# michelerenzullo/Blur_algorithms

Hardware: AMD Instinct MI355X
Metric: megapixels/sec Gaussian blur (σ=20, 4K RGB) at 1/2/4/8 GPUs; % HBM roofline (higher is better)
Workload: dtype f16 hi+lo operands (u8 pixels exact, taps and intermediate split in two binary16 halves), f32 accumulate

## Files before the change

blur_algorithms_amd/csrc/engine.hip:

```cpp
#include <hip/hip_runtime.h>

#include <array>
#include <cmath>
#include <cstdio>
#include <cstdlib>
#include <cstring>
#include <functional>
#include <list>
#include <map>
#include <memory>
#include <string>
#include <tuple>
#include <type_traits>
#include <vector>

#include "../../include/blur_amd.h"
#include "fast_registry.hpp"
#include "fft_engine.hpp"
#include "host_math.hpp"
#define BLUR_MX_QUIRK_KERNELS
#include "mx_registry.hpp"
#define BLUR_FX_QUIRK_KERNELS
#include "fx_registry.hpp"
#include "bx_box.hpp"
// ... 2608 lines not shown
        g.nframes = nf;
        g.aligned = ((cols & 3) == 0 && (reinterpret_cast<uintptr_t>(s) & 3) == 0) ? 1 : 0;
        int* spart = nullptr;
        float *vpart = nullptr, *qrow = nullptr, *qcol = nullptr;
        double* zpart = nullptr;
        if (p.mx_quirk) {
            spart = ctx->mx_sums;
            zpart = reinterpret_cast<double*>(ctx->mx_terms);
            vpart = reinterpret_cast<float*>(zpart + n_zpart * nf);
            qrow = vpart + n_vpart * nf;
            qcol = qrow + n_qrow * nf;
        }
        { TimedLaunch t(ctx, 0, nf);
          HIP_TRY(ctx, p.mx->row_u8(ctx->stream, s, ctx->work, p.mxt->frags_row, g, ctx->num_cus, spart, vpart)); }
        if (p.mx_quirk) {
            hipLaunchKernelGGL(mx_quirk_rows, dim3(zblocks, nf), dim3(256), 0, ctx->stream, spart, qrow, zpart, g, chunks, 8 * (p.mx->nkb - 2), p.mxt->dr);
            HIP_TRY(ctx, hipGetLastError());
            hipLaunchKernelGGL(mx_quirk_cols, dim3((g.vpitch + 255) / 256, nf), dim3(256), 0, ctx->stream, vpart, zpart, qcol, g, rblocks, zblocks, p.mxt->dr, p.mxt->dc);
            HIP_TRY(ctx, hipGetLastError());
        }
        { TimedLaunch t(ctx, 1, nf);
          HIP_TRY(ctx, p.mx->col_u8(ctx->stream, ctx->work, d, p.mxt->frags_col, g, qcol, ctx->num_cus, qrow)); }
    }
    return BLUR_OK;
}

static int run_fx_u8c3(blur_ctx* ctx, const uint8_t* d_src, uint8_t* d_dst, int nframes, int rows, int cols, const Prepared& p, float* vdump = nullptr, FwChSel chsel = 0,
                       const ChLayout* lay = nullptr, const FwFrame* ft)
{
    const size_t px = static_cast<size_t>(rows) * cols;
    if (lay && !chsel) return fail(ctx, BLUR_ERR_INVALID, "run_fx_u8c3: a layout goes with a channel selection");
    if (ft && !lay) return fail(ctx, BLUR_ERR_INVALID, "run_fx_u8c3: a frame list goes with a layout");
    const FwPitch pt = lay ? fw_pitch_of(*lay) : fw_pitch_packed(rows, cols, 3, 1);
    const uint8_t* lo = d_src < d_dst ? d_src : d_dst;
    const uint8_t* hi = d_src < d_dst ? d_dst : d_src;
    if (!lay && static_cast<size_t>(hi - lo) < px * 3 * nframes) {
        const size_t cap = std::max<size_t>(1, (static_cast<size_t>(1) << 30) / (px * 3));
        if (d_src == d_dst && static_cast<size_t>(nframes) > cap) {
            for (int f0 = 0; f0 < nframes; f0 += static_cast<int>(cap)) {
                const int nf = std::min<int>(static_cast<int>(cap), nframes - f0);
                if (int rc = run_fx_u8c3(ctx, d_src + static_cast<size_t>(f0) * px * 3, d_dst + static_cast<size_t>(f0) * px * 3, nf, rows, cols, p, vdump, chsel)) return rc;
            }
            return BLUR_OK;
        }
        if (int rc = ensure_work(ctx, px * 3 * nframes)) return rc;
        HIP_TRY(ctx, hipMemcpyAsync(ctx->work, d_src, px * 3 * nframes, hipMemcpyDeviceToDevice, ctx->stream));
        d_src = reinterpret_cast<const uint8_t*>(ctx->work);
    }
    const int nkb = p.fx->nkb, pada = 8 * (nkb - 2);
    FxGeom g{ rows, cols, p.sz.pad, nframes, 0, (rows + 31) / 32, fx_right_strips(cols, pada), ctx->num_xcds };
    g.aligned = ((cols & 3) == 0 && (reinterpret_cast<uintptr_t>(d_src) & 3) == 0 && (reinterpret_cast<uintptr_t>(d_dst) & 3) == 0) ? 1 : 0;
    {
        const int win = kFxChunk + 2 * pada, nstrips = fx_left_strips(pada) + g.nright;
        const size_t bytes = static_cast<size_t>(nframes) * nstrips * rows * win * 3 + 64;
        if (ctx->fx_strips_bytes < bytes) {
            if (ctx->fx_strips) { HIP_TRY(ctx, hipStreamSynchronize(ctx->stream)); HIP_TRY(ctx, hipFree(ctx->fx_strips)); ctx->fx_strips = nullptr; ctx->fx_strips_bytes = 0; }
            HIP_TRY(ctx, hipMalloc(reinterpret_cast<void**>(&ctx->fx_strips), bytes));
            ctx->fx_strips_bytes = bytes;
        }
    }
    const int chunks_x = (cols + kFxChunk - 1) / kFxChunk, narrow =
#ifdef FX_FULL_STRIPS
        0;
#else
        p.fx->nkb <= 11 && !chsel ? 1 : 0;
#endif
    int strip_groups = (kFxChunk + 2 * pada) / 4;
    if (narrow) {
        const int gpr = strip_groups, per = (gpr + 7) / 8, nleft = fx_left_strips(pada);
        strip_groups = 0;
        for (int si = 0; si < nleft + g.nright; ++si) {
            int lo, hi;
            fx_strip_range(si < nleft ? si : chunks_x - g.nright + si - nleft, cols, pada, per, &lo, &hi);
            strip_groups = std::max(strip_groups, std::min(8 * hi, gpr) - 8 * lo);
        }
        if (strip_groups < 1) strip_groups = 1;
    }
    const int strip_blocks = (((rows + 3) / 4) * strip_groups + 255) / 256;
    const int n_strip = strip_blocks * (fx_left_strips(pada) + g.nright) * nframes;
    FxQuirk qk{};
    if (!p.mx_quirk) {
        TimedLaunch t(ctx, 1, nframes);
        if (ft)
            hipLaunchKernelGGL(fx_prepass_frames<1>, dim3(n_strip), dim3(256), 0, ctx->stream, d_src, nullptr, nullptr, nullptr, ctx->fx_strips, rows, cols, pada, 1, 1, 0,
                               chunks_x, g.nright, strip_blocks, kFxSumRows, narrow, pt.src_pitch, pt.src_frame, ft);
        else
            hipLaunchKernelGGL(fx_prepass<1>, dim3(n_strip), dim3(256), 0, ctx->stream, d_src, nullptr, nullptr, nullptr, ctx->fx_strips, rows, cols, p.sz.pad, pada, 1, 1, 0,
                               chunks_x, g.nright, strip_blocks, kFxSumRows, narrow, pt.src_pitch, pt.src_frame);
        HIP_TRY(ctx, hipGetLastError());
    }
    if (p.mx_quirk) {
        const int gpt = fx_groups_per_thread(cols);
        const int groups = (cols + 3) / 4;
        const int band_rows = fx_band_rows(rows, cols, nframes, ctx->num_cus), nbands = (rows + band_rows - 1) / band_rows, nbatches = (groups + 256 * gpt - 1) / (256 * gpt);
        auto up4 = [](size_t v) { return (v + 3) & ~static_cast<size_t>(3); };
        const size_t n_srow = up4(static_cast<size_t>(nframes) * nbatches * rows * 3), n_cpart = up4(static_cast<size_t>(nframes) * nbands * 12 * groups);
        const size_t n_z = static_cast<size_t>(nframes) * nbands * nbatches * 3;
        const size_t bytes = (n_srow + n_cpart) * sizeof(int) + n_z * sizeof(long long) + 64;
        if (ctx->fx_sums_bytes < bytes) {
            if (ctx->fx_sums) { HIP_TRY(ctx, hipStreamSynchronize(ctx->stream)); HIP_TRY(ctx, hipFree(ctx->fx_sums)); ctx->fx_sums = nullptr; ctx->fx_sums_bytes = 0; }
            HIP_TRY(ctx, hipMalloc(reinterpret_cast<void**>(&ctx->fx_sums), bytes + bytes / 8));
            ctx->fx_sums_bytes = bytes + bytes / 8;
        }
        int* srow = ctx->fx_sums;
        int* cpart = srow + n_srow;
        long long* zpart = reinterpret_cast<long long*>(cpart + n_cpart);
        { TimedLaunch t(ctx, 1, nframes);
          const int n_alt = nbands * nbatches * nframes;
          auto kern = gpt == 1 ? fx_prepass<1> : (gpt == 2 ? fx_prepass<2> : fx_prepass<4>);
          auto kern_frames = gpt == 1 ? fx_prepass_frames<1> : (gpt == 2 ? fx_prepass_frames<2> : fx_prepass_frames<4>);
          if (ft)
              hipLaunchKernelGGL(kern_frames, dim3(n_alt + n_strip), dim3(256), 0, ctx->stream, d_src, srow, cpart, zpart, ctx->fx_strips, rows, cols, pada, nbands, nbatches,
                                 n_alt, chunks_x, g.nright, strip_blocks, band_rows, narrow, pt.src_pitch, pt.src_frame, ft);
          else
              hipLaunchKernelGGL(kern, dim3(n_alt + n_strip), dim3(256), 0, ctx->stream, d_src, srow, cpart, zpart, ctx->fx_strips, rows, cols, p.sz.pad, pada, nbands,
                                 nbatches, n_alt, chunks_x, g.nright, strip_blocks, band_rows, narrow, pt.src_pitch, pt.src_frame);
          HIP_TRY(ctx, hipGetLastError()); }
        qk.srow_part = srow;
        qk.cpart = cpart;
        qk.zpart = zpart;
        qk.taps = p.mxt->taps_row;
        qk.nbatches = nbatches;
        qk.nbands = nbands;
        qk.cpitch = 12 * groups;
        qk.dr = p.mxt->dr;
        qk.dc = p.mxt->dc;
    }
    unsigned long long* stamps = nullptr;
    if (!p.mx_quirk && !vdump && std::getenv("BLUR_FX_STAMPS")) {
        HIP_TRY(ctx, hipMalloc(reinterpret_cast<void**>(&stamps), 64));
        HIP_TRY(ctx, hipMemset(stamps, 0, 64));
    }
    if (chsel) {
        const Fw3Entry* fe3 = find_fw3_entry(nkb);
        if (!fe3 || vdump || stamps) return fail(ctx, BLUR_ERR_UNSUPPORTED, "fused kernel for a subset of three channels: no kernel instantiated for this pad");
        TimedLaunch t(ctx, 0, nframes);
        HIP_TRY(ctx, fe3->blur_u8(ctx->stream, d_src, d_dst, p.mxt->frags_row, g, ctx->num_cus, p.mx_quirk ? &qk : nullptr, ctx->fx_strips, chsel, pt, ft));
        return BLUR_OK;
    }
    { TimedLaunch t(ctx, 0, nframes);
      HIP_TRY(ctx, p.fx->blur_u8(ctx->stream, d_src, d_dst, p.mxt->frags_row, g, ctx->num_cus, p.mx_quirk ? &qk : nullptr, ctx->fx_strips, vdump, stamps)); }
    if (stamps) {
        unsigned long long h[8];
        HIP_TRY(ctx, hipStreamSynchronize(ctx->stream));
        HIP_TRY(ctx, hipMemcpy(h, stamps, 64, hipMemcpyDeviceToHost));
        HIP_TRY(ctx, hipFree(stamps));
        if (h[7]) {
            std::fprintf(stderr, "fx stamps: steps %llu, cycles per step: A0 %.0f B0 %.0f A1 %.0f B1 %.0f A2 %.0f B2 %.0f, whole task %.0f per step\n", h[7], h[0] / double(h[7]),
                         h[1] / double(h[7]), h[2] / double(h[7]), h[3] / double(h[7]), h[4] / double(h[7]), h[5] / double(h[7]), h[6] / double(h[7]));
        }
    }
    return BLUR_OK;
}

static bool bands_overlap(const uint8_t* lo, const uint8_t* hi, size_t bytes) { return static_cast<size_t>(hi - lo) < bytes; }

static int run_wr_tiled(blur_ctx* ctx, const uint8_t* d_src, uint8_t* d_dst, int nframes, int rows, int cols, const Prepared& p)
{
    const size_t px = static_cast<size_t>(rows) * cols, fb = px * 3;
    const int pad = p.sz.pad;
    const int groups = (cols + 3) / 4, gpt = 1;
    if (p.tl_quirk && cols < 4) return fail(ctx, BLUR_ERR_UNSUPPORTED, "tiled wave-resident path: image narrower than 4 pixels (the quirk's pre-pass)");
    const int pitch = (cols + 7) & ~7;
    int *srow = nullptr, *cpart = nullptr;
    long long* zpart = nullptr;
    float *e = nullptr, *h = nullptr;
    int band_rows = 0, nbands = 0, nbatches = 0;
    if (p.tl_quirk) {
        band_rows = static_cast<long long>(rows) * cols < 4000000ll ? 16 : kFxSumRows;
        while (band_rows < 256 && static_cast<long long>((groups + 255) / 256) * ((rows + 2 * band_rows - 1) / (2 * band_rows)) >= 4ll * ctx->num_cus) band_rows *= 2;
        nbands = (rows + band_rows - 1) / band_rows;
        nbatches = (groups + 256 * gpt - 1) / (256 * gpt);
        auto up4 = [](size_t v) { return (v + 3) & ~static_cast<size_t>(3); };
        const size_t n_srow = up4(static_cast<size_t>(nbatches) * rows * 3), n_cpart = up4(static_cast<size_t>(nbands) * 12 * groups);
        const size_t n_z = static_cast<size_t>(nbands) * nbatches * 3;
        const size_t bytes = (n_srow + n_cpart) * sizeof(int) + n_z * sizeof(long long) + 64;
        if (ctx->tl_sums_bytes < bytes) {
            if (ctx->tl_sums) { HIP_TRY(ctx, hipStreamSynchronize(ctx->stream)); HIP_TRY(ctx, hipFree(ctx->tl_sums)); ctx->tl_sums = nullptr; ctx->tl_sums_bytes = 0; }
            HIP_TRY(ctx, hipMalloc(reinterpret_cast<void**>(&ctx->tl_sums), bytes));
            ctx->tl_sums_bytes = bytes;
        }
        srow = ctx->tl_sums;
        cpart = srow + n_srow;
        zpart = reinterpret_cast<long long*>(cpart + n_cpart);
        const size_t tbytes = (static_cast<size_t>(3) * pitch + static_cast<size_t>(3) * rows) * sizeof(float) + 64;
        if (ctx->tl_terms_bytes < tbytes) {
            if (ctx->tl_terms) { HIP_TRY(ctx, hipStreamSynchronize(ctx->stream)); HIP_TRY(ctx, hipFree(ctx->tl_terms)); ctx->tl_terms = nullptr; ctx->tl_terms_bytes = 0; }
            HIP_TRY(ctx, hipMalloc(reinterpret_cast<void**>(&ctx->tl_terms), tbytes));
            ctx->tl_terms_bytes = tbytes;
        }
        e = ctx->tl_terms;
        h = e + static_cast<size_t>(3) * pitch;
    }
    for (int f = 0; f < nframes; ++f) {
        const uint8_t* src = d_src + static_cast<size_t>(f) * fb;
        uint8_t* dst = d_dst + static_cast<size_t>(f) * fb;
        const uint8_t* lo = src < dst ? src : dst;
        const uint8_t* hi = src < dst ? dst : src;
        if (bands_overlap(lo, hi, fb) && (p.bands.size() > 1 || p.tiles.size() > 1 || src == dst)) {
            if (ctx->tl_copy_bytes < fb) {
                if (ctx->tl_copy) { HIP_TRY(ctx, hipStreamSynchronize(ctx->stream)); HIP_TRY(ctx, hipFree(ctx->tl_copy)); ctx->tl_copy = nullptr; ctx->tl_copy_bytes = 0; }
                HIP_TRY(ctx, hipMalloc(reinterpret_cast<void**>(&ctx->tl_copy), fb));
                ctx->tl_copy_bytes = fb;
            }
            HIP_TRY(ctx, hipMemcpyAsync(ctx->tl_copy, src, fb, hipMemcpyDeviceToDevice, ctx->stream));
            src = ctx->tl_copy;
        }
        if (p.tl_quirk) {
            TimedLaunch t(ctx, 1, 1);
            const int n_alt = nbands * nbatches;
            hipLaunchKernelGGL(fx_prepass<1>, dim3(n_alt), dim3(256), 0, ctx->stream, src, srow, cpart, zpart, nullptr, rows, cols, pad, 0, nbands, nbatches, n_alt, 1, 0, 1, band_rows, 0,
                               static_cast<uint32_t>(cols) * 3u, static_cast<size_t>(rows) * cols * 3);
            HIP_TRY(ctx, hipGetLastError());
            const int ne = (pitch + 255) / 256, nh = (rows + 255) / 256;
            const size_t lds = (static_cast<size_t>(3) * (256 + 2 * pad) + (2 * pad + 1) + 3 + 3 * 256) * sizeof(double);
            if (lds > 64 * 1024) HIP_TRY(ctx, hipFuncSetAttribute(reinterpret_cast<const void*>(tl_terms_kernel), hipFuncAttributeMaxDynamicSharedMemorySize, static_cast<int>(lds)));
            hipLaunchKernelGGL(tl_terms_kernel, dim3(ne + nh, 1), dim3(256), lds, ctx->stream, srow, cpart, zpart, p.tl_taps, e, h, rows, cols, pad, pitch, nbatches, nbands,
                               12 * groups, p.tl_dr, p.tl_dc, ne);
            HIP_TRY(ctx, hipGetLastError());
        }
        auto group_of = [&](size_t bi, int& step) -> int {
            const Prepared::Span& b = p.bands[bi];
            const int brows = b.in1 - b.in0;
            int nb = 1;
            step = 0;
            if (b.padmode == 0) {
                while (bi + nb < p.bands.size()) {
                    const Prepared::Span& c = p.bands[bi + nb];
                    const int st = c.in0 - p.bands[bi + nb - 1].in0;
                    if (c.padmode != 0 || c.in1 - c.in0 != brows || c.v0 - c.in0 != b.v0 - b.in0 || c.v1 - c.v0 != b.v1 - b.v0 || (st & 1) || (nb > 1 && st != step)) break;
                    step = st;
                    ++nb;
                }
            }
            if (nb > 1 && wr_frame_floats(brows, cols, b.padmode, p.tl_col->g) * nb * sizeof(float) > (static_cast<size_t>(3) << 30)) { nb = 1; step = 0; }
            return nb;
        };
        {
            size_t need = 0;
            for (size_t bi = 0; bi < p.bands.size();) {
                int step;
                const int nb = group_of(bi, step);
                need = std::max(need, wr_frame_floats(p.bands[bi].in1 - p.bands[bi].in0, cols, p.bands[bi].padmode, p.tl_col->g) * nb * sizeof(float));
                bi += nb;
            }
            if (int rc = ensure_work(ctx, need)) return rc;
        }
        float* const inter = reinterpret_cast<float*>(ctx->work);
        for (size_t bi = 0; bi < p.bands.size();) {
            const Prepared::Span& b = p.bands[bi];
            const int brows = b.in1 - b.in0;
            int step = 0;
            const int nb = group_of(bi, step);
            const int vr_max = bi + nb < p.bands.size() ? p.bands[bi + nb].v0 : rows;
            WrColTerm term;
            if (p.tl_quirk) {
                term.e = e;
                term.pitch = pitch;
                term.sign = ((b.in0 + pad - b.padmode) & 1) ? -1.f : 1.f;
            }
            term.band_step = nb > 1 ? step : 0;
            { TimedLaunch t(ctx, 1, 1);
              HIP_TRY(ctx, p.tl_col->col_u8(ctx->stream, src + static_cast<size_t>(b.in0) * cols * 3, inter, brows, cols, b.padmode, nb, ctx->num_cus, ctx->d_w256, p.tl_tw0_col,
                                            p.tl_m_col, term)); }
            const int g = p.tl_col->g, npairs = wr_npairs(brows, b.padmode), strips_full = (cols + g - 1) / g;
            for (size_t ti = 0; ti < p.tiles.size(); ++ti) {
                const Prepared::Span& t = p.tiles[ti];
                WrRowTile tile;
                tile.h = p.tl_quirk ? h : nullptr;
                tile.rows_full = rows;
                tile.row_base = b.in0;
                tile.vr0 = b.v0;
                tile.vr1 = b.v1;
                tile.ypar = b.padmode & 1;
                tile.dst_pitch = cols * 3;
                tile.dst_x0 = t.in0;
                tile.vc0 = t.v0 - t.in0;
                tile.vc1 = t.v1 - t.in0;
                tile.xpar = (t.in0 + pad) & 1;
                tile.plane_strips = strips_full;
                tile.g = g;
                tile.t0 = (b.v0 - b.in0 + tile.ypar) >> 1;
                tile.tn = ((b.v1 - 1 - b.in0 + tile.ypar) >> 1) - tile.t0 + 1;
                tile.band_step = nb > 1 ? step : 0;
                tile.vr_max = vr_max;
                if (nb == 1 && tile.vr1 > vr_max) tile.vr1 = vr_max;
                TimedLaunch tl(ctx, 0, 1);
                HIP_TRY(ctx, p.tl_row[ti]->row_u8(ctx->stream, inter + static_cast<size_t>(t.in0 / g) * npairs * (2 * g), dst, brows, t.in1 - t.in0, t.padmode, nb, ctx->num_cus,
                                                  ctx->d_w256, p.tl_tw0_row[ti], p.tl_m_row[ti], tile));
            }
            bi += nb;
        }
    }
    return BLUR_OK;
// ... 1353 lines not shown
```

blur_algorithms_amd/csrc/fw_kernels.hpp:

```cpp
#pragma once
#include "fx_kernels.hpp"
#include <cstddef>
#include <type_traits>

#ifndef FW_TL_REGS
#define FW_TL_REGS 12
#endif

namespace blur_amd {

typedef uint32_t FwChSel;
constexpr FwChSel fw_chsel_all(int ch) { return static_cast<FwChSel>(ch) | (ch > 1 ? 0xe40u : 0u); }
inline FwChSel fw_chsel_mask(unsigned mask, int ch)
{
    FwChSel s = 0;
    int n = 0;
    for (int c = 0; c < ch; ++c)
        if (mask >> c & 1u) s |= static_cast<FwChSel>(c) << (4 + 2 * n++);
    return s | static_cast<FwChSel>(n);
}
__host__ __device__ constexpr int fw_chsel_count(FwChSel s) { return static_cast<int>(s & 7u); }
inline unsigned fw_chsel_bits(FwChSel s)
{
    unsigned m = 0;
// ... 567 lines not shown
                for (int j = 0; j < G; ++j)
                    d[i][j] = __builtin_amdgcn_raw_buffer_load_b32(rimg, dj[j] < ndw ? roff + 4u * dj[j] - back[j] : 0xfffffff0u, 0, 0) >> (8 * back[j]);
            }
#pragma unroll
            for (int i = 0; i < RB; ++i) {
                const int r = rb + i;
                if (r >= re) break;
                const int wy = mx_alt_weight(r, rows, pad);
                int s[CH];
#pragma unroll
                for (int ch = 0; ch < CH; ++ch) s[ch] = 0;
#pragma unroll
                for (int j = 0; j < G; ++j)
#pragma unroll
                    for (int k = 0; k < 4; ++k) {
                        const int v = wx[j][k] != 0 ? static_cast<int>((d[i][j] >> (8 * k)) & 0xffu) : 0;
                        s[CH == 1 ? 0 : k % CH] += wx[j][k] * v;
                        col[j][k] += wy * v;
                    }
#pragma unroll
                for (int ch = 0; ch < CH; ++ch)
                    if (chmask >> ch & 1u) atomicAdd(&sred[r - rs][ch][tid & 63], s[ch]);
            }
        }
        __syncthreads();
        if (tid < (re - rs) * CH && (chmask >> (tid % CH) & 1u)) {
            const int rr = tid / CH, ch = tid - rr * CH;
            const int* p64 = &sred[rr][ch][0];
            int v = 0;
#pragma unroll 8
            for (int k = 0; k < 64; ++k) v += p64[(k + tid) & 63];
            atomicAdd(&srow[(static_cast<size_t>(f) * rows + rs + rr) * CH + ch], v);
            atomicAdd(reinterpret_cast<unsigned long long*>(&zsum[static_cast<size_t>(f) * CH + ch]),
                      static_cast<unsigned long long>(static_cast<long long>(mx_alt_weight(rs + rr, rows, pad)) * v));
        }
        __syncthreads();
    }
#pragma unroll
    for (int j = 0; j < G; ++j)
        if (4 * dj[j] < cpitch)
            *reinterpret_cast<int4*>(cpart + (static_cast<size_t>(f) * nbands + band) * cpitch + 4 * dj[j]) = make_int4(col[j][0], col[j][1], col[j][2], col[j][3]);
}

template <int CH, int G>
__global__ __launch_bounds__(256) void fc_prepass(const uint8_t* __restrict__ src, int* __restrict__ srow, int* __restrict__ cpart, long long* __restrict__ zsum,
                                                  uint8_t* __restrict__ strips, int rows, int cols, int pad, int pada, int nbands, int nbatches, int cpitch, int n_alt,
                                                  int chunks, int nright, int strip_blocks, int band_rows, unsigned chmask, uint32_t spitch, size_t sframe)
{
    __shared__ int sred[kFcSumRows][CH][64];
    int b = blockIdx.x;
    if (b < n_alt) {
        const int band = b % nbands, batch = (b / nbands) % nbatches, f = b / (nbands * nbatches);
        fc_altsums_body<CH, G>(src, srow, cpart, zsum, rows, cols, pad, nbands, cpitch, band, batch, f, sred, band_rows, chmask, spitch, sframe);
    } else {
        b -= n_alt;
        const int nstrips = fx_left_strips(pada) + nright, bx = b % strip_blocks, sidx = (b / strip_blocks) % nstrips, f = b / (strip_blocks * nstrips);
        fc_edge_strips_body<CH>(src, strips, rows, cols, pada, chunks, nright, bx, sidx, f, spitch, sframe);
    }
}

template <int CH, int G>
__global__ __launch_bounds__(256) void fc_prepass_frames(const uint8_t* __restrict__ src, int* __restrict__ srow, int* __restrict__ cpart, long long* __restrict__ zsum,
                                                         uint8_t* __restrict__ strips, int rows, int cols, int pada, int nbands, int nbatches, int cpitch, int n_alt,
                                                         int chunks, int nright, int strip_blocks, int band_rows, unsigned chmask, uint32_t spitch, size_t sframe,
                                                         const FwFrame* __restrict__ ft)
{
    __shared__ int sred[kFcSumRows][CH][64];
    int b = blockIdx.x;
    if (b < n_alt) {
        const int band = b % nbands, batch = (b / nbands) % nbatches, f = b / (nbands * nbatches);
        const uint8_t* s = src + (static_cast<ptrdiff_t>(ft[f].frame) - f) * static_cast<ptrdiff_t>(sframe);
        fc_altsums_body<CH, G>(s, srow, cpart, zsum, rows, cols, ft[f].pad, nbands, cpitch, band, batch, f, sred, band_rows, chmask, spitch, sframe);
    } else {
        b -= n_alt;
        const int nstrips = fx_left_strips(pada) + nright, bx = b % strip_blocks, sidx = (b / strip_blocks) % nstrips, f = b / (strip_blocks * nstrips);
        const uint8_t* s = src + (static_cast<ptrdiff_t>(ft[f].frame) - f) * static_cast<ptrdiff_t>(sframe);
        fc_edge_strips_body<CH>(s, strips, rows, cols, pada, chunks, nright, bx, sidx, f, spitch, sframe);
    }
}

#ifdef BLUR_FX_QUIRK_KERNELS
template <int G>
__global__ __launch_bounds__(256) void fx_prepass_frames(const uint8_t* __restrict__ src, int* __restrict__ srow_part, int* __restrict__ cpart, long long* __restrict__ zpart,
                                                         uint8_t* __restrict__ strips, int rows, int cols, int pada, int nbands, int nbatches, int n_alt, int chunks,
                                                         int nright, int strip_blocks, int band_rows, int narrow, uint32_t spitch, size_t sframe,
                                                         const FwFrame* __restrict__ ft)
{
    __shared__ int sred[kFxSumRows][3][64];
    int b = blockIdx.x;
    if (b < n_alt) {
        const int band = b % nbands, batch = (b / nbands) % nbatches, f = b / (nbands * nbatches);
        const uint8_t* s = src + (static_cast<ptrdiff_t>(ft[f].frame) - f) * static_cast<ptrdiff_t>(sframe);
        fx_altsums_body<G>(s, srow_part, cpart, zpart, rows, cols, ft[f].pad, nbands, nbatches, band, batch, f, sred, band_rows, spitch, sframe);
    } else {
        b -= n_alt;
        const int nstrips = fx_left_strips(pada) + nright, bx = b % strip_blocks, sidx = (b / strip_blocks) % nstrips, f = b / (strip_blocks * nstrips);
        const uint8_t* s = src + (static_cast<ptrdiff_t>(ft[f].frame) - f) * static_cast<ptrdiff_t>(sframe);
        fx_edge_strips_body(s, strips, rows, cols, pada, chunks, nright, bx, sidx, f, narrow, spitch, sframe);
    }
}
#endif

}
```

blur_algorithms_amd/csrc/fx_kernels.hpp:

```cpp
#pragma once
#include "mx_kernels.hpp"
#include <atomic>

#if !defined(FX_NO_SGB) && !defined(FX_SGB)
#define FX_SGB 1
#endif
#ifndef FX_SGB_A
#define FX_SGB_A 5
#endif
#ifndef FX_SGB_B
#define FX_SGB_B 6
#endif

namespace blur_amd {

struct FxGeom {
    int rows, cols, pad;
    int nframes;
    int aligned;
    int ntiles;
    int nright;
    int nxcd;
};

// ... 589 lines not shown
        for (int qs = 0; qs < NT; ++qs) {
            const int s = sb + qs;
            if (s >= s1) break;
            step(s, qs, -1);
        }
    }
    store_tile(s1 - 1 - NT, s1 - 1 - NT >= tile0);
#ifdef FX_STAMPS
    if (!QUIRK && !DUMPV && vdump && blockIdx.x == 0 && tid == 0) {
        unsigned long long* o = reinterpret_cast<unsigned long long*>(vdump);
        for (int i = 0; i < 6; ++i) o[i] = st_acc[i];
        o[6] = __builtin_amdgcn_s_memtime() - st_begin;
        o[7] = static_cast<unsigned long long>(s1 - s0);
    }
#endif
}

#ifdef BLUR_FX_QUIRK_KERNELS
inline int fx_right_strips(int cols, int pada)
{
    const int chunks = (cols + kFxChunk - 1) / kFxChunk;
    int n = 0;
    for (int xc = chunks - 1; xc >= fx_left_strips(pada) && kFxChunk * xc + kFxChunk + pada > cols; --xc) ++n;
    return n;
}

__device__ __forceinline__ void fx_edge_strips_body(const uint8_t* __restrict__ src, uint8_t* __restrict__ strips, int rows, int cols, int pada, int chunks, int nright,
                                                    int bx, int sidx, int f, int narrow, uint32_t spitch, size_t sframe)
{
    const int win = kFxChunk + 2 * pada, gpr = win / 4;
    const int nleft = fx_left_strips(pada);
    const int xc = sidx < nleft ? sidx : chunks - nright + sidx - nleft, x0 = kFxChunk * xc;
    int glo = 0, gn = gpr;
    if (narrow) {
        int lo, hi;
        fx_strip_range(xc, cols, pada, (gpr + 7) / 8, &lo, &hi);
        glo = 8 * lo;
        gn = min(8 * hi, gpr) - glo;
    }
    const int i = bx * 256 + threadIdx.x, rq = (rows + 3) / 4;
    if (i >= rq * gn) return;
    const int r4 = i / gn, gidx = glo + i - r4 * gn;
    const int X = x0 - pada + 4 * gidx;
    const bool mir = X < 0 || X >= cols;
    const int xs = X < 0 ? -X - 3 : (X >= cols ? 2 * cols - 5 - X : X);
    const bool fast = xs >= 0 && xs + 3 < cols;
    typedef uint32_t u3 __attribute__((ext_vector_type(3)));
    const uint8_t* img = src + static_cast<size_t>(f) * sframe;
    uint8_t* sbase = strips + (static_cast<size_t>(f) * (nleft + nright) + sidx) * rows * (3 * win) + 12 * gidx;
    u3 d[4];
    if (fast) {
#pragma unroll
        for (int k = 0; k < 4; ++k) d[k] = *reinterpret_cast<const u3*>(img + static_cast<size_t>(min(4 * r4 + k, rows - 1)) * spitch + 3 * xs);
    }
#pragma unroll
    for (int k = 0; k < 4; ++k) {
        const int r = 4 * r4 + k;
        if (r >= rows) break;
        u3 o;
        if (fast) {
            o = d[k];
            if (mir) {
                o[0] = __builtin_amdgcn_perm(d[k][2], d[k][1], 0x02070605u);
                o[1] = (d[k][1] >> 24) | ((d[k][2] & 0xffu) << 8) | ((d[k][0] >> 24) << 16) | ((d[k][1] & 0xffu) << 24);
                o[2] = __builtin_amdgcn_perm(d[k][1], d[k][0], 0x02010005u);
            }
        } else {
            const uint8_t* line = img + static_cast<size_t>(r) * spitch;
            uint32_t b[12];
#pragma unroll
            for (int qd = 0; qd < 4; ++qd) {
                const uint8_t* px = line + 3 * mx_refl(X + qd, cols);
                b[3 * qd] = px[0]; b[3 * qd + 1] = px[1]; b[3 * qd + 2] = px[2];
            }
            o[0] = b[0] | (b[1] << 8) | (b[2] << 16) | (b[3] << 24);
            o[1] = b[4] | (b[5] << 8) | (b[6] << 16) | (b[7] << 24);
            o[2] = b[8] | (b[9] << 8) | (b[10] << 16) | (b[11] << 24);
        }
        *reinterpret_cast<u3*>(sbase + static_cast<size_t>(r) * (3 * win)) = o;
    }
}

constexpr int kFxSumRows = 32;
inline int fx_groups_per_thread(int cols)
{
    const int groups = (cols + 3) / 4;
    for (int g = 1; g <= 4; g *= 2)
        if (groups <= 256 * g * kFxMaxBatches) return g;
    return 0;
}
inline int fx_band_rows(int rows, int cols, int nframes, int num_cus)
{
    if (static_cast<long long>(rows) * cols < 4000000ll) return 16;
    const int gpt = fx_groups_per_thread(cols);
    const long long nbatches = ((cols + 3) / 4 + 256 * gpt - 1) / (256 * (gpt > 0 ? gpt : 1));
    int br = kFxSumRows;
#ifndef FX_BAND_WGS
#define FX_BAND_WGS 4
#endif
    while (br < 128 && nbatches * ((rows + 2 * br - 1) / (2 * br)) * nframes >= static_cast<long long>(FX_BAND_WGS) * num_cus) br *= 2;
    return br;
}

template <int G>
__device__ __forceinline__ void fx_altsums_body(const uint8_t* __restrict__ src, int* __restrict__ srow_part, int* __restrict__ cpart, long long* __restrict__ zpart,
                                                int rows, int cols, int pad, int nbands, int nbatches, int band, int batch, int f, int (*sred)[3][64], int band_rows,
                                                uint32_t spitch, size_t sframe)
{
    const int tid = threadIdx.x;
    const uint8_t* img = src + static_cast<size_t>(f) * sframe;
    const __amdgpu_buffer_rsrc_t rimg = __builtin_amdgcn_make_buffer_rsrc(const_cast<uint8_t*>(img), 0, static_cast<uint32_t>(rows - 1) * spitch + static_cast<uint32_t>(cols) * 3u, kMxRsrcWord3);
    const int groups = (cols + 3) / 4, r0 = band * band_rows, r1 = min(r0 + band_rows, rows);
    const int flip = (pad & 1) ? -1 : 1;
    const int over = (4 - (cols & 3)) & 3;
    int gi[G], wq[G][4];
    bool act[G], plain[G], last[G];
    uint32_t col0[G];
#pragma unroll
    for (int j = 0; j < G; ++j) {
        gi[j] = (batch * G + j) * 256 + tid;
        act[j] = gi[j] < groups;
        last[j] = over != 0 && gi[j] == groups - 1;
        const int x = 4 * gi[j] - (last[j] ? over : 0);
        plain[j] = !last[j] && x > pad && x + 3 < cols - 1 - pad;
#pragma unroll
        for (int q = 0; q < 4; ++q) wq[j][q] = (act[j] && !(last[j] && q < over)) ? mx_alt_weight(x + q, cols, pad) : 0;
        col0[j] = act[j] ? 3u * static_cast<uint32_t>(x) : 0u;
    }
    int o[G][12];
#pragma unroll
    for (int j = 0; j < G; ++j)
#pragma unroll
        for (int k = 0; k < 12; ++k) o[j][k] = 0;
    long long zacc = 0;
    typedef uint32_t u3 __attribute__((ext_vector_type(3)));
    for (int rs = r0; rs < r1; rs += kFxSumRows) {
        const int re = min(rs + kFxSumRows, r1);
        for (int i = tid; i < kFxSumRows * 3 * 64; i += 256) (&sred[0][0][0])[i] = 0;
        __syncthreads();
        uint32_t accp[G][6], accn[G][6];
#pragma unroll
        for (int j = 0; j < G; ++j)
#pragma unroll
            for (int k = 0; k < 6; ++k) accp[j][k] = accn[j][k] = 0;
#ifndef FX_PRE_RB
#define FX_PRE_RB 8
#endif
        constexpr int RB = G == 1 ? FX_PRE_RB : (G == 2 ? 4 : 2);
        for (int rb = rs; rb < re; rb += RB) {
            u3 d[RB][G];
#pragma unroll
            for (int i = 0; i < RB; ++i) {
                const int r = min(rb + i, re - 1);
#pragma unroll
                for (int j = 0; j < G; ++j) d[i][j] = __builtin_amdgcn_raw_buffer_load_b96(rimg, col0[j] + static_cast<uint32_t>(r) * spitch, 0, 0);
            }
#pragma unroll
            for (int i = 0; i < RB; ++i) {
                const int r = rb + i;
                if (r < re) {
                    const int wy = mx_alt_weight(r, rows, pad);
                    const uint32_t aw = static_cast<uint32_t>(wy < 0 ? -wy : wy);
                    int s[3] = { 0, 0, 0 };
#pragma unroll
                    for (int j = 0; j < G; ++j) {
                        const u3 dd = d[i][j];
                        if (plain[j]) {
                            const int e0 = static_cast<int>(dd[0] ^ 0x80808080u), e1 = static_cast<int>(dd[1] ^ 0x80808080u), e2 = static_cast<int>(dd[2] ^ 0x80808080u);
                            int t0 = __builtin_amdgcn_sdot4(e0, static_cast<int>(0xff000001u), 0, false);
                            t0 = __builtin_amdgcn_sdot4(e1, 0x00010000, t0, false);
                            t0 = __builtin_amdgcn_sdot4(e2, 0x0000ff00, t0, false);
                            int t1 = __builtin_amdgcn_sdot4(e0, 0x00000100, 0, false);
                            t1 = __builtin_amdgcn_sdot4(e1, 0x010000ff, t1, false);
                            t1 = __builtin_amdgcn_sdot4(e2, 0x00ff0000, t1, false);
                            int t2 = __builtin_amdgcn_sdot4(e0, 0x00010000, 0, false);
                            t2 = __builtin_amdgcn_sdot4(e1, 0x0000ff00, t2, false);
                            t2 = __builtin_amdgcn_sdot4(e2, static_cast<int>(0xff000001u), t2, false);
                            s[0] += flip * t0; s[1] += flip * t1; s[2] += flip * t2;
                        } else {
#pragma unroll
                            for (int q = 0; q < 4; ++q)
#pragma unroll
                                for (int c = 0; c < 3; ++c) {
                                    const int byte = 3 * q + c;
                                    s[c] += wq[j][q] * static_cast<int>((dd[byte >> 2] >> (8 * (byte & 3))) & 0xffu);
                                }
                        }
#pragma unroll
                        for (int k = 0; k < 3; ++k) {
                            uint32_t lo = __builtin_amdgcn_perm(0u, dd[k], 0x0c020c00u), hi = __builtin_amdgcn_perm(0u, dd[k], 0x0c030c01u);
                            if (aw != 1) { lo *= aw; hi *= aw; }
                            if (wy > 0) { accp[j][2 * k] += lo; accp[j][2 * k + 1] += hi; }
                            else { accn[j][2 * k] += lo; accn[j][2 * k + 1] += hi; }
                        }
                    }
#pragma unroll
                    for (int c = 0; c < 3; ++c) atomicAdd(&sred[r - rs][c][tid & 63], s[c]);
                }
            }
        }
#pragma unroll
        for (int j = 0; j < G; ++j)
#pragma unroll
            for (int k = 0; k < 3; ++k) {
                o[j][4 * k] += static_cast<int>(accp[j][2 * k] & 0xffffu) - static_cast<int>(accn[j][2 * k] & 0xffffu);
                o[j][4 * k + 2] += static_cast<int>(accp[j][2 * k] >> 16) - static_cast<int>(accn[j][2 * k] >> 16);
                o[j][4 * k + 1] += static_cast<int>(accp[j][2 * k + 1] & 0xffffu) - static_cast<int>(accn[j][2 * k + 1] & 0xffffu);
                o[j][4 * k + 3] += static_cast<int>(accp[j][2 * k + 1] >> 16) - static_cast<int>(accn[j][2 * k + 1] >> 16);
            }
        __syncthreads();
        if (tid < (re - rs) * 3) {
            const int* p64 = &sred[0][0][0] + 64 * tid;
            int v = 0;
#pragma unroll 8
            for (int k = 0; k < 64; ++k) v += p64[(k + tid) & 63];
            srow_part[((static_cast<size_t>(f) * nbatches + batch) * rows + rs) * 3 + tid] = v;
            zacc += static_cast<long long>(mx_alt_weight(rs + tid / 3, rows, pad)) * v;
        }
        __syncthreads();
    }
    if (over != 0) {
#pragma unroll
        for (int j = 0; j < G; ++j)
#pragma unroll
            for (int k = 0; k < 9; ++k) {
                const int v3 = o[j][k + 3], v6 = k + 6 < 12 ? o[j][k + 6] : 0, v9 = k + 9 < 12 ? o[j][k + 9] : 0;
                o[j][k] = last[j] ? (over == 1 ? v3 : (over == 2 ? v6 : v9)) : o[j][k];
            }
    }
#pragma unroll
    for (int j = 0; j < G; ++j)
        if (act[j]) {
            int4* dstp = reinterpret_cast<int4*>(cpart + (static_cast<size_t>(f) * nbands + band) * (12 * static_cast<size_t>(groups)) + 12 * gi[j]);
            dstp[0] = make_int4(o[j][0], o[j][1], o[j][2], o[j][3]);
            dstp[1] = make_int4(o[j][4], o[j][5], o[j][6], o[j][7]);
            dstp[2] = make_int4(o[j][8], o[j][9], o[j][10], o[j][11]);
        }
    long long* zs = reinterpret_cast<long long*>(&sred[0][0][0]);
    if (tid < 96) zs[tid] = zacc;
    __syncthreads();
    if (tid < 3) {
        long long z = 0;
        for (int k = 0; k < kFxSumRows; ++k) z += zs[3 * k + tid];
        zpart[((static_cast<size_t>(f) * nbands + band) * nbatches + batch) * 3 + tid] = z;
    }
}

template <int G>
__global__ __launch_bounds__(256) void fx_prepass(const uint8_t* __restrict__ src, int* __restrict__ srow_part, int* __restrict__ cpart, long long* __restrict__ zpart,
                                                  uint8_t* __restrict__ strips, int rows, int cols, int pad, int pada, int nbands, int nbatches, int n_alt, int chunks,
                                                  int nright, int strip_blocks, int band_rows, int narrow, uint32_t spitch, size_t sframe)
{
    __shared__ int sred[kFxSumRows][3][64];
    int b = blockIdx.x;
    if (b < n_alt) {
        const int band = b % nbands, batch = (b / nbands) % nbatches, f = b / (nbands * nbatches);
        fx_altsums_body<G>(src, srow_part, cpart, zpart, rows, cols, pad, nbands, nbatches, band, batch, f, sred, band_rows, spitch, sframe);
    } else {
        b -= n_alt;
        const int nstrips = fx_left_strips(pada) + nright, bx = b % strip_blocks, sidx = (b / strip_blocks) % nstrips, f = b / (strip_blocks * nstrips);
        fx_edge_strips_body(src, strips, rows, cols, pada, chunks, nright, bx, sidx, f, narrow, spitch, sframe);
    }
}
#endif

struct FxLaunch {
    int chunks = 0, nseg = 1, tps = 0;
    long long ntasks = 0;
    dim3 grid;
};
inline FxLaunch fx_plan_launch(FxGeom& g, int nch, int nt, int num_cus)
{
    FxLaunch l;
    l.chunks = (g.cols + kFxChunk - 1) / kFxChunk;
    const long long nstripes = static_cast<long long>(l.chunks) * g.nframes * nch;
    if (nstripes <= 0) return l;
    l.tps = g.ntiles;
    long long best = -1;
    for (int n = 1; n <= g.ntiles; ++n) {
        const int t = (g.ntiles + n - 1) / n, ns = (g.ntiles + t - 1) / t;
        const long long rounds = (nstripes * ns + num_cus - 1) / num_cus, span = rounds * (t + nt);
        if (best < 0 || span < best) { best = span; l.nseg = ns; l.tps = t; }
    }
    l.ntasks = nstripes * l.nseg;
    if (g.nxcd < 1) g.nxcd = 1;
    const int per_xcd = static_cast<int>((l.ntasks + g.nxcd - 1) / g.nxcd);
    l.grid = dim3(static_cast<unsigned>(g.nxcd * per_xcd));
    return l;
}

template <class... K> hipError_t fx_set_lds(std::atomic<unsigned long long>& done, int lds, K... kernels)
{
    int dev = -1;
    const bool known = hipGetDevice(&dev) == hipSuccess && dev >= 0 && dev < 64;
    if (known && ((done.load(std::memory_order_acquire) >> dev) & 1ull)) return hipSuccess;
    for (const void* k : { reinterpret_cast<const void*>(kernels)... }) {
        const hipError_t e = hipFuncSetAttribute(k, hipFuncAttributeMaxDynamicSharedMemorySize, lds);
        if (e != hipSuccess) return e;
    }
    if (known) done.fetch_or(1ull << dev, std::memory_order_release);
    return hipSuccess;
}

struct FxEntry {
    int nkb;
    hipError_t (*blur_u8)(hipStream_t, const uint8_t* src, uint8_t* dst, const void* frags, FxGeom g, int num_cus, const FxQuirk* qk, const uint8_t* strips,
                          float* vdump, unsigned long long* stamps);
};

template <int NKB> hipError_t fx_launch_u8(hipStream_t st, const uint8_t* src, uint8_t* dst, const void* frags, FxGeom g, int num_cus, const FxQuirk* qk,
                                           const uint8_t* strips, float* vdump, unsigned long long* stamps)
{
    using C = FxCfg<NKB>;
    const FxLaunch l = fx_plan_launch(g, 1, C::NT, num_cus);
    if (l.ntasks == 0) return hipSuccess;
    static std::atomic<unsigned long long> attr_done{ 0 };
    const hipError_t e = fx_set_lds(attr_done, C::LDS, fx_blur_u8<NKB, true, false>, fx_blur_u8<NKB, false, false>, fx_blur_u8<NKB, true, true>,
                                    fx_blur_u8<NKB, false, true>, fx_blur_u8<NKB, true, false, true>, fx_blur_u8<NKB, false, false, true>);
    if (e != hipSuccess) return e;
#define FX_LAUNCH(Q_, D_, R_)                                                                                                                              \
    hipLaunchKernelGGL((fx_blur_u8<NKB, Q_, D_, R_>), l.grid, dim3(256), C::LDS, st, src, dst, static_cast<const mx_half8*>(frags), g, l.chunks, l.tps, \
                       l.nseg, static_cast<int>(l.ntasks), qk ? *qk : FxQuirk{}, strips, vdump ? vdump : reinterpret_cast<float*>(stamps))
    const bool ragged = (g.cols & 3) != 0;
    if (vdump) {
        if (ragged) return hipErrorNotSupported;
        if (qk) FX_LAUNCH(true, true, false); else FX_LAUNCH(false, true, false);
    } else if (ragged) { if (qk) FX_LAUNCH(true, false, true); else FX_LAUNCH(false, false, true); }
    else { if (qk) FX_LAUNCH(true, false, false); else FX_LAUNCH(false, false, false); }
#undef FX_LAUNCH
    return hipGetLastError();
}

#define BLUR_FX(NKB_)                                                                                       \
    namespace blur_amd {                                                                                    \
    const FxEntry* fx_entry_##NKB_()                                                                        \
    {                                                                                                       \
        static const FxEntry e = { NKB_, fx_launch_u8<NKB_> };                                              \
        return &e;                                                                                          \
    }                                                                                                       \
    }
// ... 3 lines not shown
```

Baseline: 195,400.

## Restructure alt-sums prepass with register prefetch ring and double-buffered LDS reductions

```diff
diff --git a/blur_algorithms_amd/csrc/engine.hip b/blur_algorithms_amd/csrc/engine.hip
--- a/blur_algorithms_amd/csrc/engine.hip
+++ b/blur_algorithms_amd/csrc/engine.hip
@@ -2714,10 +2714,10 @@
     if (!p.mx_quirk) {
         TimedLaunch t(ctx, 1, nframes);
         if (ft)
-            hipLaunchKernelGGL(fx_prepass_frames<1>, dim3(n_strip), dim3(256), 0, ctx->stream, d_src, nullptr, nullptr, nullptr, ctx->fx_strips, rows, cols, pada, 1, 1, 0,
+            hipLaunchKernelGGL(fx_prepass_frames<1>, dim3(n_strip), dim3(256), 0, ctx->stream, d_src, nullptr, nullptr, nullptr, ctx->fx_strips, rows, cols, pada, 1, 1, 0, 0,
                                chunks_x, g.nright, strip_blocks, kFxSumRows, narrow, pt.src_pitch, pt.src_frame, ft);
         else
-            hipLaunchKernelGGL(fx_prepass<1>, dim3(n_strip), dim3(256), 0, ctx->stream, d_src, nullptr, nullptr, nullptr, ctx->fx_strips, rows, cols, p.sz.pad, pada, 1, 1, 0,
+            hipLaunchKernelGGL(fx_prepass<1>, dim3(n_strip), dim3(256), 0, ctx->stream, d_src, nullptr, nullptr, nullptr, ctx->fx_strips, rows, cols, p.sz.pad, pada, 1, 1, 0, 0,
                                chunks_x, g.nright, strip_blocks, kFxSumRows, narrow, pt.src_pitch, pt.src_frame);
         HIP_TRY(ctx, hipGetLastError());
     }
@@ -2725,6 +2725,7 @@
         const int gpt = fx_groups_per_thread(cols);
         const int groups = (cols + 3) / 4;
         const int band_rows = fx_band_rows(rows, cols, nframes, ctx->num_cus), nbands = (rows + band_rows - 1) / band_rows, nbatches = (groups + 256 * gpt - 1) / (256 * gpt);
+        const int bw = fx_batch_groups(groups, nbatches);
         auto up4 = [](size_t v) { return (v + 3) & ~static_cast<size_t>(3); };
         const size_t n_srow = up4(static_cast<size_t>(nframes) * nbatches * rows * 3), n_cpart = up4(static_cast<size_t>(nframes) * nbands * 12 * groups);
         const size_t n_z = static_cast<size_t>(nframes) * nbands * nbatches * 3;
@@ -2743,10 +2744,10 @@
           auto kern_frames = gpt == 1 ? fx_prepass_frames<1> : (gpt == 2 ? fx_prepass_frames<2> : fx_prepass_frames<4>);
           if (ft)
               hipLaunchKernelGGL(kern_frames, dim3(n_alt + n_strip), dim3(256), 0, ctx->stream, d_src, srow, cpart, zpart, ctx->fx_strips, rows, cols, pada, nbands, nbatches,
-                                 n_alt, chunks_x, g.nright, strip_blocks, band_rows, narrow, pt.src_pitch, pt.src_frame, ft);
+                                 bw, n_alt, chunks_x, g.nright, strip_blocks, band_rows, narrow, pt.src_pitch, pt.src_frame, ft);
           else
               hipLaunchKernelGGL(kern, dim3(n_alt + n_strip), dim3(256), 0, ctx->stream, d_src, srow, cpart, zpart, ctx->fx_strips, rows, cols, p.sz.pad, pada, nbands,
-                                 nbatches, n_alt, chunks_x, g.nright, strip_blocks, band_rows, narrow, pt.src_pitch, pt.src_frame);
+                                 nbatches, bw, n_alt, chunks_x, g.nright, strip_blocks, band_rows, narrow, pt.src_pitch, pt.src_frame);
           HIP_TRY(ctx, hipGetLastError()); }
         qk.srow_part = srow;
         qk.cpart = cpart;
@@ -2841,7 +2842,8 @@
         if (p.tl_quirk) {
             TimedLaunch t(ctx, 1, 1);
             const int n_alt = nbands * nbatches;
-            hipLaunchKernelGGL(fx_prepass<1>, dim3(n_alt), dim3(256), 0, ctx->stream, src, srow, cpart, zpart, nullptr, rows, cols, pad, 0, nbands, nbatches, n_alt, 1, 0, 1, band_rows, 0,
+            hipLaunchKernelGGL(fx_prepass<1>, dim3(n_alt), dim3(256), 0, ctx->stream, src, srow, cpart, zpart, nullptr, rows, cols, pad, 0, nbands, nbatches,
+                               fx_batch_groups(groups, nbatches), n_alt, 1, 0, 1, band_rows, 0,
                                static_cast<uint32_t>(cols) * 3u, static_cast<size_t>(rows) * cols * 3);
             HIP_TRY(ctx, hipGetLastError());
             const int ne = (pitch + 255) / 256, nh = (rows + 255) / 256;
diff --git a/blur_algorithms_amd/csrc/fw_kernels.hpp b/blur_algorithms_amd/csrc/fw_kernels.hpp
--- a/blur_algorithms_amd/csrc/fw_kernels.hpp
+++ b/blur_algorithms_amd/csrc/fw_kernels.hpp
@@ -673,16 +673,16 @@
 #ifdef BLUR_FX_QUIRK_KERNELS
 template <int G>
 __global__ __launch_bounds__(256) void fx_prepass_frames(const uint8_t* __restrict__ src, int* __restrict__ srow_part, int* __restrict__ cpart, long long* __restrict__ zpart,
-                                                         uint8_t* __restrict__ strips, int rows, int cols, int pada, int nbands, int nbatches, int n_alt, int chunks,
-                                                         int nright, int strip_blocks, int band_rows, int narrow, uint32_t spitch, size_t sframe,
+                                                         uint8_t* __restrict__ strips, int rows, int cols, int pada, int nbands, int nbatches, int bw, int n_alt,
+                                                         int chunks, int nright, int strip_blocks, int band_rows, int narrow, uint32_t spitch, size_t sframe,
                                                          const FwFrame* __restrict__ ft)
 {
-    __shared__ int sred[kFxSumRows][3][64];
+    __shared__ __attribute__((aligned(8))) int sred[kFxRedInts];
     int b = blockIdx.x;
     if (b < n_alt) {
         const int band = b % nbands, batch = (b / nbands) % nbatches, f = b / (nbands * nbatches);
         const uint8_t* s = src + (static_cast<ptrdiff_t>(ft[f].frame) - f) * static_cast<ptrdiff_t>(sframe);
-        fx_altsums_body<G>(s, srow_part, cpart, zpart, rows, cols, ft[f].pad, nbands, nbatches, band, batch, f, sred, band_rows, spitch, sframe);
+        fx_altsums_body<G>(s, srow_part, cpart, zpart, rows, cols, ft[f].pad, nbands, nbatches, bw, band, batch, f, sred, band_rows, spitch, sframe);
     } else {
         b -= n_alt;
         const int nstrips = fx_left_strips(pada) + nright, bx = b % strip_blocks, sidx = (b / strip_blocks) % nstrips, f = b / (strip_blocks * nstrips);
diff --git a/blur_algorithms_amd/csrc/fx_kernels.hpp b/blur_algorithms_amd/csrc/fx_kernels.hpp
--- a/blur_algorithms_amd/csrc/fx_kernels.hpp
+++ b/blur_algorithms_amd/csrc/fx_kernels.hpp
@@ -695,6 +695,9 @@
 }
 
 constexpr int kFxSumRows = 32;
+constexpr int kFxRedRows = 16;
+constexpr int kFxRedPitch = 65;
+constexpr int kFxRedInts = kFxSumRows * 3 * kFxRedPitch;
 inline int fx_groups_per_thread(int cols)
 {
     const int groups = (cols + 3) / 4;
@@ -702,6 +705,7 @@
         if (groups <= 256 * g * kFxMaxBatches) return g;
     return 0;
 }
+inline int fx_batch_groups(int groups, int nbatches) { return (groups + nbatches - 1) / nbatches; }
 inline int fx_band_rows(int rows, int cols, int nframes, int num_cus)
 {
     if (static_cast<long long>(rows) * cols < 4000000ll) return 16;
@@ -715,63 +719,76 @@
     return br;
 }
 
+__device__ __forceinline__ void fx_lds_barrier()
+{
+    __builtin_amdgcn_fence(__ATOMIC_RELEASE, "workgroup", "local");
+    __builtin_amdgcn_s_barrier();
+    __builtin_amdgcn_fence(__ATOMIC_ACQUIRE, "workgroup", "local");
+}
+
 template <int G>
 __device__ __forceinline__ void fx_altsums_body(const uint8_t* __restrict__ src, int* __restrict__ srow_part, int* __restrict__ cpart, long long* __restrict__ zpart,
-                                                int rows, int cols, int pad, int nbands, int nbatches, int band, int batch, int f, int (*sred)[3][64], int band_rows,
-                                                uint32_t spitch, size_t sframe)
-{
+                                                int rows, int cols, int pad, int nbands, int nbatches, int bw, int band, int batch, int f, int* sred,
+                                                int band_rows, uint32_t spitch, size_t sframe)
+{
+    static_assert(kFxSumRows == 2 * kFxRedRows, "two buffers of row sums per flush of the packed column sums");
     const int tid = threadIdx.x;
     const uint8_t* img = src + static_cast<size_t>(f) * sframe;
     const __amdgpu_buffer_rsrc_t rimg = __builtin_amdgcn_make_buffer_rsrc(const_cast<uint8_t*>(img), 0, static_cast<uint32_t>(rows - 1) * spitch + static_cast<uint32_t>(cols) * 3u, kMxRsrcWord3);
+    constexpr uint32_t kOutside = 0xfffffff0u;
     const int groups = (cols + 3) / 4, r0 = band * band_rows, r1 = min(r0 + band_rows, rows);
-    const int flip = (pad & 1) ? -1 : 1;
+    const bool flip = (pad & 1) != 0;
+    const int wA = flip ? 0x010000ff : static_cast<int>(0xff000001u), wB = flip ? 0x00ff0000 : 0x00010000, wC = flip ? 0x00000100 : 0x0000ff00;
+    const int nA = flip ? static_cast<int>(0xff000001u) : 0x010000ff, nB = flip ? 0x00010000 : 0x00ff0000, nC = flip ? 0x0000ff00 : 0x00000100;
     const int over = (4 - (cols & 3)) & 3;
     int gi[G], wq[G][4];
     bool act[G], plain[G], last[G];
     uint32_t col0[G];
 #pragma unroll
     for (int j = 0; j < G; ++j) {
-        gi[j] = (batch * G + j) * 256 + tid;
-        act[j] = gi[j] < groups;
+        gi[j] = batch * bw + j * 256 + tid;
+        act[j] = j * 256 + tid < bw && gi[j] < groups;
         last[j] = over != 0 && gi[j] == groups - 1;
         const int x = 4 * gi[j] - (last[j] ? over : 0);
-        plain[j] = !last[j] && x > pad && x + 3 < cols - 1 - pad;
+        plain[j] = !last[j] && (!act[j] || (x > pad && x + 3 < cols - 1 - pad));
 #pragma unroll
         for (int q = 0; q < 4; ++q) wq[j][q] = (act[j] && !(last[j] && q < over)) ? mx_alt_weight(x + q, cols, pad) : 0;
-        col0[j] = act[j] ? 3u * static_cast<uint32_t>(x) : 0u;
+        col0[j] = 3u * static_cast<uint32_t>(x);
     }
     int o[G][12];
 #pragma unroll
     for (int j = 0; j < G; ++j)
 #pragma unroll
         for (int k = 0; k < 12; ++k) o[j][k] = 0;
+    uint32_t acc[2][G][6];
+#pragma unroll
+    for (int j = 0; j < G; ++j)
+#pragma unroll
+        for (int k = 0; k < 6; ++k) acc[0][j][k] = acc[1][j][k] = 0;
+    const int sgn = ((r0 + pad) & 1) ? -1 : 1;
     long long zacc = 0;
     typedef uint32_t u3 __attribute__((ext_vector_type(3)));
-    for (int rs = r0; rs < r1; rs += kFxSumRows) {
-        const int re = min(rs + kFxSumRows, r1);
-        for (int i = tid; i < kFxSumRows * 3 * 64; i += 256) (&sred[0][0][0])[i] = 0;
-        __syncthreads();
-        uint32_t accp[G][6], accn[G][6];
-#pragma unroll
-        for (int j = 0; j < G; ++j)
-#pragma unroll
-            for (int k = 0; k < 6; ++k) accp[j][k] = accn[j][k] = 0;
 #ifndef FX_PRE_RB
 #define FX_PRE_RB 8
 #endif
-        constexpr int RB = G == 1 ? FX_PRE_RB : (G == 2 ? 4 : 2);
-        for (int rb = rs; rb < re; rb += RB) {
-            u3 d[RB][G];
-#pragma unroll
-            for (int i = 0; i < RB; ++i) {
-                const int r = min(rb + i, re - 1);
-#pragma unroll
-                for (int j = 0; j < G; ++j) d[i][j] = __builtin_amdgcn_raw_buffer_load_b96(rimg, col0[j] + static_cast<uint32_t>(r) * spitch, 0, 0);
-            }
+    constexpr int RB = G == 1 ? FX_PRE_RB : (G == 2 ? 4 : 2);
+    static_assert(kFxRedRows % RB == 0 && RB % 2 == 0, "a ring slot always holds the same row of a trip, even slots even rows");
+    u3 d[RB][G];
+#pragma unroll
+    for (int i = 0; i < RB; ++i)
+#pragma unroll
+        for (int j = 0; j < G; ++j)
+            d[i][j] = __builtin_amdgcn_raw_buffer_load_b96(rimg, (act[j] && r0 + i < r1) ? col0[j] + static_cast<uint32_t>(r0 + i) * spitch : kOutside, 0, 0);
+    for (int i = tid; i < kFxRedInts; i += 256) sred[i] = 0;
+    fx_lds_barrier();
+    for (int hs = r0, half = 0; hs < r1; hs += kFxRedRows, half ^= 1) {
+        const int he = min(hs + kFxRedRows, r1);
+        int* red = sred + half * (kFxRedRows * 3 * kFxRedPitch);
+        for (int rb = hs; rb < he; rb += RB) {
 #pragma unroll
             for (int i = 0; i < RB; ++i) {
                 const int r = rb + i;
-                if (r < re) {
+                if (r < r1) {
                     const int wy = mx_alt_weight(r, rows, pad);
                     const uint32_t aw = static_cast<uint32_t>(wy < 0 ? -wy : wy);
                     int s[3] = { 0, 0, 0 };
@@ -780,16 +797,15 @@
                         const u3 dd = d[i][j];
                         if (plain[j]) {
                             const int e0 = static_cast<int>(dd[0] ^ 0x80808080u), e1 = static_cast<int>(dd[1] ^ 0x80808080u), e2 = static_cast<int>(dd[2] ^ 0x80808080u);
-                            int t0 = __builtin_amdgcn_sdot4(e0, static_cast<int>(0xff000001u), 0, false);
-                            t0 = __builtin_amdgcn_sdot4(e1, 0x00010000, t0, false);
-                            t0 = __builtin_amdgcn_sdot4(e2, 0x0000ff00, t0, false);
-                            int t1 = __builtin_amdgcn_sdot4(e0, 0x00000100, 0, false);
-                            t1 = __builtin_amdgcn_sdot4(e1, 0x010000ff, t1, false);
-                            t1 = __builtin_amdgcn_sdot4(e2, 0x00ff0000, t1, false);
-                            int t2 = __builtin_amdgcn_sdot4(e0, 0x00010000, 0, false);
-                            t2 = __builtin_amdgcn_sdot4(e1, 0x0000ff00, t2, false);
-                            t2 = __builtin_amdgcn_sdot4(e2, static_cast<int>(0xff000001u), t2, false);
-                            s[0] += flip * t0; s[1] += flip * t1; s[2] += flip * t2;
+                            s[0] = __builtin_amdgcn_sdot4(e0, wA, s[0], false);
+                            s[0] = __builtin_amdgcn_sdot4(e1, wB, s[0], false);
+                            s[0] = __builtin_amdgcn_sdot4(e2, wC, s[0], false);
+                            s[1] = __builtin_amdgcn_sdot4(e0, nC, s[1], false);
+                            s[1] = __builtin_amdgcn_sdot4(e1, nA, s[1], false);
+                            s[1] = __builtin_amdgcn_sdot4(e2, nB, s[1], false);
+                            s[2] = __builtin_amdgcn_sdot4(e0, wB, s[2], false);
+                            s[2] = __builtin_amdgcn_sdot4(e1, wC, s[2], false);
+                            s[2] = __builtin_amdgcn_sdot4(e2, wA, s[2], false);
                         } else {
 #pragma unroll
                             for (int q = 0; q < 4; ++q)
@@ -801,36 +817,52 @@
                         }
 #pragma unroll
                         for (int k = 0; k < 3; ++k) {
-                            uint32_t lo = __builtin_amdgcn_perm(0u, dd[k], 0x0c020c00u), hi = __builtin_amdgcn_perm(0u, dd[k], 0x0c030c01u);
-                            if (aw != 1) { lo *= aw; hi *= aw; }
-                            if (wy > 0) { accp[j][2 * k] += lo; accp[j][2 * k + 1] += hi; }
-                            else { accn[j][2 * k] += lo; accn[j][2 * k + 1] += hi; }
+                            const uint32_t lo = __builtin_amdgcn_perm(0u, dd[k], 0x0c020c00u), hi = __builtin_amdgcn_perm(0u, dd[k], 0x0c030c01u);
+                            acc[i & 1][j][2 * k] += __umul24(lo, aw);
+                            acc[i & 1][j][2 * k + 1] += __umul24(hi, aw);
                         }
                     }
 #pragma unroll
-                    for (int c = 0; c < 3; ++c) atomicAdd(&sred[r - rs][c][tid & 63], s[c]);
+                    for (int c = 0; c < 3; ++c) atomicAdd(&red[((r - hs) * 3 + c) * kFxRedPitch + (tid & 63)], s[c]);
                 }
-            }
-        }
-#pragma unroll
-        for (int j = 0; j < G; ++j)
-#pragma unroll
-            for (int k = 0; k < 3; ++k) {
-                o[j][4 * k] += static_cast<int>(accp[j][2 * k] & 0xffffu) - static_cast<int>(accn[j][2 * k] & 0xffffu);
-                o[j][4 * k + 2] += static_cast<int>(accp[j][2 * k] >> 16) - static_cast<int>(accn[j][2 * k] >> 16);
-                o[j][4 * k + 1] += static_cast<int>(accp[j][2 * k + 1] & 0xffffu) - static_cast<int>(accn[j][2 * k + 1] & 0xffffu);
-                o[j][4 * k + 3] += static_cast<int>(accp[j][2 * k + 1] >> 16) - static_cast<int>(accn[j][2 * k + 1] >> 16);
-            }
-        __syncthreads();
-        if (tid < (re - rs) * 3) {
-            const int* p64 = &sred[0][0][0] + 64 * tid;
-            int v = 0;
-#pragma unroll 8
-            for (int k = 0; k < 64; ++k) v += p64[(k + tid) & 63];
-            srow_part[((static_cast<size_t>(f) * nbatches + batch) * rows + rs) * 3 + tid] = v;
-            zacc += static_cast<long long>(mx_alt_weight(rs + tid / 3, rows, pad)) * v;
-        }
-        __syncthreads();
+                const int rn = r + RB;
+#pragma unroll
+                for (int j = 0; j < G; ++j)
+                    d[i][j] = __builtin_amdgcn_raw_buffer_load_b96(rimg, (act[j] && rn < r1) ? col0[j] + static_cast<uint32_t>(rn) * spitch : kOutside, 0, 0);
+            }
+        }
+        if (half || he == r1) {
+#pragma unroll
+            for (int j = 0; j < G; ++j)
+#pragma unroll
+                for (int k = 0; k < 3; ++k) {
+                    const uint32_t e0 = acc[0][j][2 * k], e1 = acc[0][j][2 * k + 1], o0 = acc[1][j][2 * k], o1 = acc[1][j][2 * k + 1];
+                    o[j][4 * k] += sgn * (static_cast<int>(e0 & 0xffffu) - static_cast<int>(o0 & 0xffffu));
+                    o[j][4 * k + 2] += sgn * (static_cast<int>(e0 >> 16) - static_cast<int>(o0 >> 16));
+                    o[j][4 * k + 1] += sgn * (static_cast<int>(e1 & 0xffffu) - static_cast<int>(o1 & 0xffffu));
+                    o[j][4 * k + 3] += sgn * (static_cast<int>(e1 >> 16) - static_cast<int>(o1 >> 16));
+                    acc[0][j][2 * k] = acc[0][j][2 * k + 1] = acc[1][j][2 * k] = acc[1][j][2 * k + 1] = 0;
+                }
+        }
+        fx_lds_barrier();
+        {
+            const int v = tid >> 2, qd = tid & 3;
+            int sum = 0;
+            if (tid < 4 * 3 * kFxRedRows) {
+                int* p16 = red + kFxRedPitch * v + 16 * qd;
+#pragma unroll
+                for (int k = 0; k < 16; ++k) {
+                    sum += p16[k];
+                    p16[k] = 0;
+                }
+            }
+            sum += __shfl_xor(sum, 1, 64);
+            sum += __shfl_xor(sum, 2, 64);
+            if (qd == 0 && v < (he - hs) * 3) {
+                srow_part[((static_cast<size_t>(f) * nbatches + batch) * rows + hs) * 3 + v] = sum;
+                zacc += static_cast<long long>(mx_alt_weight(hs + v / 3, rows, pad)) * sum;
+            }
+        }
     }
     if (over != 0) {
 #pragma unroll
@@ -849,26 +881,27 @@
             dstp[1] = make_int4(o[j][4], o[j][5], o[j][6], o[j][7]);
             dstp[2] = make_int4(o[j][8], o[j][9], o[j][10], o[j][11]);
         }
-    long long* zs = reinterpret_cast<long long*>(&sred[0][0][0]);
-    if (tid < 96) zs[tid] = zacc;
-    __syncthreads();
+    fx_lds_barrier();
+    long long* zs = reinterpret_cast<long long*>(sred);
+    zs[tid] = zacc;
+    fx_lds_barrier();
     if (tid < 3) {
         long long z = 0;
-        for (int k = 0; k < kFxSumRows; ++k) z += zs[3 * k + tid];
+        for (int k = 0; k < kFxRedRows; ++k) z += zs[4 * (3 * k + tid)];
         zpart[((static_cast<size_t>(f) * nbands + band) * nbatches + batch) * 3 + tid] = z;
     }
 }
 
 template <int G>
 __global__ __launch_bounds__(256) void fx_prepass(const uint8_t* __restrict__ src, int* __restrict__ srow_part, int* __restrict__ cpart, long long* __restrict__ zpart,
-                                                  uint8_t* __restrict__ strips, int rows, int cols, int pad, int pada, int nbands, int nbatches, int n_alt, int chunks,
-                                                  int nright, int strip_blocks, int band_rows, int narrow, uint32_t spitch, size_t sframe)
-{
-    __shared__ int sred[kFxSumRows][3][64];
+                                                  uint8_t* __restrict__ strips, int rows, int cols, int pad, int pada, int nbands, int nbatches, int bw, int n_alt,
+                                                  int chunks, int nright, int strip_blocks, int band_rows, int narrow, uint32_t spitch, size_t sframe)
+{
+    __shared__ __attribute__((aligned(8))) int sred[kFxRedInts];
     int b = blockIdx.x;
     if (b < n_alt) {
         const int band = b % nbands, batch = (b / nbands) % nbatches, f = b / (nbands * nbatches);
-        fx_altsums_body<G>(src, srow_part, cpart, zpart, rows, cols, pad, nbands, nbatches, band, batch, f, sred, band_rows, spitch, sframe);
+        fx_altsums_body<G>(src, srow_part, cpart, zpart, rows, cols, pad, nbands, nbatches, bw, band, batch, f, sred, band_rows, spitch, sframe);
     } else {
         b -= n_alt;
         const int nstrips = fx_left_strips(pada) + nright, bx = b % strip_blocks, sidx = (b / strip_blocks) % nstrips, f = b / (strip_blocks * nstrips);
```

After: 199,100 (median of 6 runs). 1.9% higher.
